# sleep3r/Diffusion-Handwriting-Generation.pytorch

Hardware: AMD Instinct MI355X
Metric: stroke-points/sec reverse-sampled (T=60, L=488) (higher is better)
Workload: dtype bf16; 1 GPU; configs[1]: batch=64 prompts/GPU, T=60, L=488, Lt=30, d_model=128/192/256, num_layers=2, diffusion_mode=new, random-init weights; global_batch=64, seq_len=488, parallelism=batch-shard x1 (no collectives)

## Files before the change

### diffusion-handwriting-generation.pytorch_amd/csrc/convblock_core.h

```cpp
#pragma once
#include <algorithm>
#include "enc_a_core.h"
#include "heads_core.h"

namespace {

#define CB_SILU(x) ((DHW_ABL & 8) ? (x) : silu_t<T>(x))
#define CB_SILU_TILES(NT_, MT_, v) do { if constexpr (!(DHW_ABL & 8)) silu_tiles2<T, NT_, MT_>(v); } while (0)
#define CB_BARRIER() do { if constexpr (!(DHW_ABL & 64)) lds_barrier(); } while (0)

#define STAMP(slot) DHW_STAMP_IF(p.stamps && (int)blockIdx.x == p.stagger && (threadIdx.x & 63) == 0, (threadIdx.x >> 6) * 16 + slot, __builtin_amdgcn_s_memrealtime())

template <typename T, int BM> __host__ __device__ constexpr int h2_stride(int CO) { return BM >= 128 ? CO * (int)sizeof(T) + 16 : tile_stride<T>(CO); }

template <int NT>
struct Epi {
  f32x4 bias[NT], gam[NT], bet[NT];
  DHW_DEV void load(const float* b, const float* g, const float* be, int n0) {
#pragma unroll
    for (int i = 0; i < NT; ++i) {
      bias[i] = *reinterpret_cast<const f32x4*>(b + n0 + 16 * i);
      gam[i] = *reinterpret_cast<const f32x4*>(g + n0 + 16 * i);
      bet[i] = *reinterpret_cast<const f32x4*>(be + n0 + 16 * i);
    }
// ... 4 lines not shown
      bias[i] = *reinterpret_cast<const f32x4*>(b + n0 + 16 * i);
      gam[i] = (f32x4){1, 1, 1, 1};
      bet[i] = (f32x4){0, 0, 0, 0};
    }
  }
};

template <int UPC> constexpr int up_skip_width() { return UPC == 384 ? 256 : UPC == 256 ? 192 : UPC == 192 ? 128 : 0; }
template <typename T, int BM, int CO, int NW, int OCC = 1, int UPC = 0, int CH = 0, int CIN = 0, int TIGHT = 0, int PP = 0, typename P, typename X>
DHW_DEV void convblock_body(const P& p, const X& nx, const int b, const int m0, char* smem) {
  constexpr int ES = sizeof(T), NTHR = NW * 64;
  constexpr bool SK = CIN != 0;
  constexpr int KT1 = 3 * CIN / 32;
  static_assert(UPC == 0 || CIN == 0 || CIN == UPC, "a fused input stage produces the block's own input width");
  constexpr bool ASYM = TIGHT == 2;
  constexpr int BMO = ASYM ? BM : BM - 2 - 2 * TIGHT;
  constexpr int RX = BMO + 4;
  constexpr int BM1 = ASYM ? BM + 16 : BM;
  constexpr int C1 = CO / 2;
  constexpr int T1 = C1 / 16, T2 = CO / 16;
  constexpr int WN1 = NW == 8 ? (T1 >= 8 ? 8 : (T1 == 6 ? 6 : 4)) : 2;
  constexpr int WM1 = NW == 8 ? (T1 >= 6 ? 1 : 2) : 2;
  constexpr bool TALL = NW == 8 && BM >= 128 && T2 == 8;
  constexpr int WN2 = NW == 8 ? (TALL ? 4 : (T2 % 8 == 0 ? 8 : 6)) : 4;
  constexpr int WM2 = TALL ? 2 : 1;
  constexpr int MT1 = BM1 / WM1 / 16, NT1 = T1 / WN1;
  constexpr int MT2 = BM / WM2 / 16, NT2 = T2 / WN2;
  static_assert(NT1 * WN1 == T1 && NT2 * WN2 == T2 && MT1 * 16 * WM1 == BM1 && WM1 * WN1 <= NW && WM2 * WN2 <= NW, "unsupported tile / wave layout");
  static_assert(!ASYM || WM1 == 1, "the asymmetric tiling: blocks with one row group in conv1");
  constexpr bool PPX = PP != 0;
  static_assert(!PPX || (TALL && WM1 == 2 && WN1 == 4 && CH == 0 && !ASYM && OCC == 1), "ping-pong: the 2 x 4 wave layouts of the tall tiles");
  constexpr int RING = (ES == 2 ? 24 : 12) * (CO == 256 ? 2 : 3) / 3 / (OCC * NW > 8 ? OCC : 1);

  const int Ls = sample_len(p.lens, p.lsh, b, p.L);
  if constexpr (DHW_LENS) { if (m0 >= Ls) return; }
  const int tid = body_tid(), lane = tid & 63, wave = __builtin_amdgcn_readfirstlane(tid >> 6);
  const int l15 = lane & 15, g = lane >> 4;
  const int Cin = SK ? CIN : p.Cin;
  const bool pp_lead = PPX && __builtin_amdgcn_readfirstlane(wave) >= NW / 2;
#define PP_BARRIER() do { if constexpr (PPX) CB_BARRIER(); } while (0)

  const int SX = tile_stride<T>(Cin), SH1 = tile_stride<T>(C1), SH2 = h2_stride<T, BM>(CO);
  char* XS = smem;
  char* XR = XS + RX * SX;
  char* H1 = XR + RX * SX;
  char* H2 = H1 + (BM1 + 2) * SH1;
  const float* gam = p.film + (size_t)b * p.film_bs;
  const float* bet = gam + p.film_tot;

  const bool act1 = WM1 * WN1 == NW || wave < WM1 * WN1, act2 = WM2 * WN2 == NW || wave < WM2 * WN2;
  const int wm1 = act1 ? wave / WN1 : 0, wn1 = act1 ? wave % WN1 : 0, row01 = wm1 * (BM1 / WM1), nt01 = wn1 * NT1;
  const int wm2 = act2 ? wave / WN2 : 0, wn2 = act2 ? wave % WN2 : 0, row02 = wm2 * (BM / WM2), nt02 = wn2 * NT2;
  const int n1 = nt01 * 16 + 4 * g, n2 = nt02 * 16 + 4 * g;
  const int KCin = Cin / 32;

  if constexpr (OCC == 2) {
    if (p.stagger && blockIdx.x >= gridDim.x / 2)
      for (int i = 0; i < p.stagger; ++i) __builtin_amdgcn_s_sleep(16);
  }
  STAMP(0);
  WRing<T, NT1, RING> ring1;
  Epi<NT1> ep1;
  auto fill1 = [&]() {
    const T* w = reinterpret_cast<const T*>(p.w_c1) + ((size_t)nt01 * KCin * 3 * 64 + lane) * 8;
    if constexpr (SK) ring1.template fill_s<KT1>(w);
    else ring1.fill(w, KCin * 3);
  };

  if constexpr (UPC != 0) {
    constexpr int RXP = (RX + 15) / 16 * 16, RH = RXP + 2, MTU = RXP / 16;
    constexpr int TU = UPC / 16, WNU = TU % 8 == 0 ? 8 : 4, WMU = NW / WNU, NTU = TU / WNU;
    constexpr int MTG = (MTU + WMU - 1) / WMU;
    static_assert(NTU * WNU == TU && NW == 8, "unsupported input width");
    const int wmu = wave / WNU, wnu = wave % WNU;
    const int ntu0 = wnu * NTU, nu = ntu0 * 16 + 4 * g, rowu0 = wmu * MTG * 16;
    constexpr int UCH = up_skip_width<UPC>();
// ... 115 lines not shown
          const bool k = lrow >= 0 && lrow < Ls;
          uint4 w = make_uint4(k ? v[u].x : 0u, k ? v[u].y : 0u, k ? v[u].z : 0u, k ? v[u].w : 0u);
          *reinterpret_cast<uint4*>(XR + r * SX + cc * 16) = w;
          *reinterpret_cast<uint4*>(XS + r * SX + cc * 16) = (DHW_ABL & 8) ? w : silu_piece<T>(w);
        }
      }
    }
  }
  if (UPC == 0 && act1) {
    fill1();
    ep1.load(p.b_c1, gam + p.f1, bet + p.f1, n1);
  }
  STAMP(15);
  CB_BARRIER();
  if constexpr (PPX) {
    if (!pp_lead) {
      for (int id = tid; id < 2 * SH1 / 16; id += NTHR / 2)
        *reinterpret_cast<uint4*>(H1 + BM1 * SH1 + id * 16) = make_uint4(0, 0, 0, 0);
      CB_BARRIER();
    }
  }
  STAMP(1);

  WRing<T, NT2, RING> ring2;
  Epi<NT2> ep2;

  {
    f32x4 acc[NT1][MT1];
    acc_zero(acc);
    if (act1) {
      if constexpr (SK) ring1.template run_s<MT1, KT1>(acc, XS + (row01 + l15) * SX + g * 8 * ES, SX, KCin);
      else ring1.template run<MT1>(acc, XS + (row01 + l15) * SX + g * 8 * ES, SX, KCin);
    }
    STAMP(2);
    PP_BARRIER();
    constexpr int KT2 = (C1 / 32) * 3;
    const T* w2 = reinterpret_cast<const T*>(p.w_c2) + ((size_t)nt02 * KT2 * 64 + lane) * 8;
    if (act2) { ring2.template fill_begin<KT2>(w2); ep2.load(p.b_c2, gam + p.f2, bet + p.f2, n2); }
    constexpr int ST1 = epilogue_steps<NT1, MT1>(), CH2 = decltype(ring2)::template fill_chunks<KT2>(), PER1 = (CH2 + ST1 - 1) / ST1;
    if (act1) {
      epilogue_pairs<T, NT1, MT1, !(DHW_ABL & 8)>(lane, H1, SH1, row01, n1, acc,
          [&](int i, const f32x4& a) { return (a + ep1.bias[i]) * ep1.gam[i] + ep1.bet[i]; },
          [&](int j) { const int srow = m0 - 1 + row01 + j * 16 + l15; return srow >= 0 && srow < Ls; },
          [](int) { return true; },
          [&](int step) {
            if (act2) {
#pragma unroll
              for (int c = 0; c < PER1; ++c) ring2.template fill_chunk<KT2>(step * PER1 + c);
            }
          });
    } else if (act2) {
#pragma unroll
      for (int c = 0; c < CH2; ++c) ring2.template fill_chunk<KT2>(c);
    }
    if constexpr (!PPX)
    for (int id = tid; id < 2 * SH1 / 16; id += NTHR)
      *reinterpret_cast<uint4*>(H1 + BM1 * SH1 + id * 16) = make_uint4(0, 0, 0, 0);
  }
  STAMP(13);
  CB_BARRIER();
  STAMP(3);

  if (act2) {
    f32x4 acc[NT2][MT2];
    acc_zero(acc);
    ring2.template run_s<MT2, (C1 / 32) * 3>(acc, H1 + (row02 + l15) * SH1 + g * 8 * ES, SH1, C1 / 32);
    STAMP(4);
    PP_BARRIER();
    {
      constexpr int KTF = CO / 32;
      ring2.template fill_begin<KTF>(reinterpret_cast<const T*>(p.w_fc) + ((size_t)nt02 * KTF * 64 + lane) * 8);
      constexpr int ST2 = epilogue_steps<NT2, MT2>(), CHF = decltype(ring2)::template fill_chunks<KTF>(), PER2 = (CHF + ST2 - 1) / ST2;
      epilogue_pairs<T, NT2, MT2, !(DHW_ABL & 8)>(lane, H2, SH2, row02, n2, acc,
          [&](int i, const f32x4& a) { return (a + ep2.bias[i]) * ep2.gam[i] + ep2.bet[i]; },
          [](int) { return true; }, [](int) { return true; },
          [&](int step) {
#pragma unroll
            for (int c = 0; c < PER2; ++c) ring2.template fill_chunk<KTF>(step * PER2 + c);
          });
    }
    ep2.load(p.b_fc, gam + p.f3, bet + p.f3, n2);
  }
  STAMP(14);
  CB_BARRIER();
  STAMP(5);

  f32x4 acc[NT2][MT2];
  acc_zero(acc);
  if (act2) {
    const T* wsk = reinterpret_cast<const T*>(p.w_skip) + ((size_t)nt02 * KCin * 3 * 64 + lane) * 8;
    constexpr bool FCX = SK && CO / 32 <= decltype(ring2)::D && DHW_ABL == 0;
    if constexpr (FCX) ring2.template run_n<MT2, CO / 32, KT1>(acc, H2 + (row02 + l15) * SH2 + g * 8 * ES, SH2, CO / 32, wsk);
    else ring2.template run_s<MT2, CO / 32>(acc, H2 + (row02 + l15) * SH2 + g * 8 * ES, SH2, CO / 32);
    STAMP(6);
    if constexpr (FCX) {}
    else if constexpr (SK) ring2.template fill_s<KT1>(wsk);
    else ring2.fill(wsk, KCin * 3);
#pragma unroll
    for (int i = 0; i < NT2; ++i)
#pragma unroll
      for (int j = 0; j < MT2; ++j) acc[i][j] = (acc[i][j] + ep2.bias[i]) * ep2.gam[i] + ep2.bet[i];
    ep2.load_bias(p.b_skip, n2);
    if constexpr (SK) ring2.template run_s<MT2, KT1>(acc, XR + (row02 + l15 + 1) * SX + g * 8 * ES, SX, KCin);
    else ring2.template run<MT2>(acc, XR + (row02 + l15 + 1) * SX + g * 8 * ES, SX, KCin);
  }
  STAMP(7);
  CB_BARRIER();
  if constexpr (PPX) { if (pp_lead && p.out_f32) CB_BARRIER(); }
  STAMP(8);

  const int rows_valid = min(BMO, Ls - m0);
  if (p.out_f32) {
    constexpr int SO = CO * 4 + 16;
    if (act2) {
#pragma unroll
      for (int i = 0; i < NT2; ++i)
#pragma unroll
        for (int j = 0; j < MT2; ++j)
          store4(reinterpret_cast<float*>(smem + (row02 + j * 16 + l15) * SO) + n2 + 16 * i, acc[i][j] + ep2.bias[i]);
    }
    CB_BARRIER();
    if (p.out)
      tile_copy_out<float>(smem, SO, reinterpret_cast<float*>(p.out) + (size_t)(b * p.L + m0) * CO, CO, rows_valid, CO, tid, NTHR);
    if (p.fuse_heads) {
      const int r = tid >> 2, q = tid & 3;
      float a0 = 0.f, a1 = 0.f, a2 = 0.f;
      if (r < rows_valid) {
        const float* xr = reinterpret_cast<const float*>(smem + r * SO);
#pragma unroll
        for (int c = q * 4; c < CO; c += 16) {
          const f32x4 v = *reinterpret_cast<const f32x4*>(xr + c);
          const f32x4 w0 = *reinterpret_cast<const f32x4*>(p.hp.w_out + c);
          const f32x4 w1 = *reinterpret_cast<const f32x4*>(p.hp.w_out + CO + c);
          const f32x4 w2 = *reinterpret_cast<const f32x4*>(p.hp.w_pen + c);
#pragma unroll
          for (int k = 0; k < 4; ++k) { a0 += v[k] * w0[k]; a1 += v[k] * w1[k]; a2 += v[k] * w2[k]; }
        }
      }
#pragma unroll
      for (int o = 2; o; o >>= 1) {
        a0 += __shfl_xor(a0, o);
        a1 += __shfl_xor(a1, o);
        a2 += __shfl_xor(a2, o);
      }
      if (r < rows_valid && q == 0) heads_finish(p.hp, (long)b * p.L + m0 + r, a0, a1, a2);
    }
  } else {
    if (act2) {
#pragma unroll
      for (int i = 0; i < NT2; ++i)
#pragma unroll
        for (int j = 0; j < MT2; ++j) acc[i][j] += ep2.bias[i];
      store_tiles<T, NT2, MT2>(lane, smem, SH2, row02, n2, acc);
    }
    CB_BARRIER();
    if constexpr (PPX) { if (pp_lead) CB_BARRIER(); }
    if constexpr (!(DHW_ABL & 16))
    tile_copy_out<T>(smem, SH2, reinterpret_cast<T*>(p.out) + (size_t)(b * p.L + m0) * CO, CO, rows_valid, CO, tid, NTHR);
    if (p.pool && !(DHW_ABL & 16))
      tile_copy_out_pool<T>(smem, SH2, reinterpret_cast<T*>(p.pool) + ((size_t)b * (p.L / 2) + m0 / 2) * CO, CO, rows_valid, CO, tid, NTHR);
    if constexpr (CH == 1) {
      static_assert(NW == 8 && sizeof(T) == 2, "enc_a_body runs on 8 waves");
      EncALds m;
      m.XR = smem;
      m.QR = smem + BM * SH2;
      m.red = reinterpret_cast<float*>(m.QR + BM * SH2);
      m.KT = reinterpret_cast<char*>(m.red) + 2 * 8 * BM * sizeof(float);
      m.VT = m.KT + 32 * tile_stride<T>(CO);
      m.VS = smem;
      m.PL = reinterpret_cast<float*>(m.KT + enc_a_text_kv_bytes<T, CO, BM>());
      enc_a_body<T, CO, BM, (ASYM ? 16 : 4)>(nx.a, m, b, m0, rows_valid);
    }
  }
  STAMP(9);
}

template <typename T, int BM, int CO>
// ... 12 lines not shown
```

### diffusion-handwriting-generation.pytorch_amd/csrc/enc_a_core.h

```cpp
#pragma once
#include "attn_core.h"
#include "gemm_core.h"
#include "dhw_kernels.h"

#define ENC_STAMP(slot) do { DHW_STAMP_IF(p.stamps && blockIdx.x == 0 && threadIdx.x == 0, slot, __builtin_amdgcn_s_memrealtime()); \
                             DHW_STAMP_IF(p.stamps && (p.dbg & 4) && blockIdx.x == 0 && (threadIdx.x & 63) == 0, 64 + (threadIdx.x >> 6) * 32 + (slot), __builtin_amdgcn_s_memtime()); } while (0)

template <typename T, int BM>
DHW_DEV void stage_rows(char* dst, int S, const T* src, int C, int b, int L, int m0, int tid, int nthreads) {
  constexpr int ES = sizeof(T);
  const int cpr = C * ES / 16;
  const int total = BM * cpr;
  constexpr int U = 4;
  for (int base = tid; base < total; base += nthreads * U) {
    uint4 v[U];
    int off[U];
#pragma unroll
    for (int u = 0; u < U; ++u) {
      const int id = base + u * nthreads;
      const int r = id / cpr, cc = id - r * cpr;
      v[u] = make_uint4(0, 0, 0, 0);
      off[u] = id < total ? r * S + cc * 16 : -1;
      if (id < total && m0 + r < L)
        v[u] = *reinterpret_cast<const uint4*>(reinterpret_cast<const char*>(src) + ((size_t)(b * L + m0 + r) * C) * ES + (size_t)cc * 16);
// ... 67 lines not shown
      if (c < W / 4 && grp + 4 < NS) *reinterpret_cast<uint4*>(pa + 4 * W) = b;
    }
  }
};
template <typename T> constexpr bool enc_plds() { return sizeof(T) == 2; }
template <typename T, int DM> constexpr size_t enc_a_param_bytes() { return enc_plds<T>() ? (size_t)7 * DM * sizeof(float) : 0; }

struct EncALds {
  char* XR;
  char* QR;
  float* red;
  char* KT;
  char* VT;
  char* VS;
  float* PL;
};
template <typename T, int DM, int BM>
constexpr size_t enc_a_text_kv_bytes() {
  return sizeof(T) == 2 ? (size_t)2 * 32 * tile_stride<T>(DM) : (size_t)32 * tile_stride<T>(DM) + (size_t)DM * (32 * sizeof(T) + OPAD<T>);
}
template <typename T, int DM> constexpr int qkv_stride() { return sizeof(T) == 2 ? 3 * DM : 2 * DM; }

template <int DM> constexpr int enc_wn() { return DM % 128 == 0 ? 8 : 6; }

template <typename T, int DM, int BM, int VPIECE = 16, typename P>
DHW_DEV void enc_a_body(const P& p, const EncALds& m, int b, int m0, int rows_valid) {
  constexpr int ES = sizeof(T);
  constexpr int WN = enc_wn<DM>(), WM = 1;
  constexpr int MT = BM / WM / 16, NT = DM / WN / 16, H = DM / 64, KC = DM / 32;
  static_assert(NT * WN * 16 == DM, "channel tiles must divide over the waves");
  const int tid = body_tid(), lane = tid & 63, wave = tid >> 6;
  const int l15 = lane & 15, g = lane >> 4;
  const bool act = WN * WM == 8 || wave < WN * WM;
  const int wm = act ? wave / WN : 0, wn = act ? wave % WN : 0;
  const int S = tile_stride<T>(DM);
  const int Ls = sample_len(p.lens, p.lsh, b, p.Lk);
  char* XR = m.XR;
  char* QR = m.QR;
  float* red = m.red;
  const float* gam = p.film + (size_t)b * p.film_bs;
  const float* bet = gam + p.film_tot;
  const int row0 = wm * (BM / WM), ntile0 = wn * NT;
  const int n0 = ntile0 * 16 + 4 * g;
  const size_t wlane = ((size_t)ntile0 * KC * 64 + lane) * 8;
  const char* xop = XR + (row0 + l15) * S + g * 8 * ES;
  const char* qop = QR + (row0 + l15) * S + g * 8 * ES;

  constexpr int RINGA = sizeof(T) == 4 ? 12 : 24;
  typedef WRing<T, NT, RINGA, (RINGA + NT - 1) / NT> RingT;
  RingT ring;
  constexpr bool SPREADA = sizeof(T) == 2;
  constexpr bool SPREADQ = sizeof(T) == 2 && MT > 1;
  constexpr int FCHA = RingT::template fill_chunks<KC>(), FQA = (FCHA + 3) / 4;
  EpiParams<NT> ep;
  ENC_STAMP(0);
  constexpr bool VROW = sizeof(T) == 2;
  constexpr int KBC = 32, SKC = tile_stride<T>(DM), SVC = VROW ? SKC : KBC * ES + OPAD<T>;
  constexpr int EPV = 16 / ES, CPR = DM / EPV, PPR = KBC / EPV;
  constexpr int UX = (BM * CPR + 511) / 512, UK = (KBC * CPR + 511) / 512, UV = VROW ? UK : (DM * PPR + 511) / 512;
  constexpr int QKS = qkv_stride<T, DM>();
  char* KT = m.KT;
  char* VT = m.VT;
  const T* k1s = reinterpret_cast<const T*>(p.k1) + (size_t)b * p.Lt * DM;
  const T* v1s = reinterpret_cast<const T*>(p.vt1) + (VROW ? (size_t)b * p.Lt * DM : (size_t)b * DM * p.lpadT);
  constexpr bool PLDS = enc_plds<T>();
  const float* PL = m.PL;
  const int64_t* trow = p.text ? p.text + (size_t)b * p.Lt : nullptr;
  PadMask<KBC> pad;
  struct KVRegs { CopyRegs<UK> ck; CopyRegs<UV> cv; };
  auto kv_store = [&](KVRegs& kv) {
    CopyRegs<UK>& ck = kv.ck;
    CopyRegs<UV>& cv = kv.cv;
    ck.store(KBC * CPR, tid, 512, [&](int id) { const int r = id / CPR, cc = id - r * CPR; return reinterpret_cast<uint4*>(KT + r * SKC + cc * 16); },
             [&](int id) { return id / CPR < p.Lt; });
    if constexpr (VROW)
      cv.store(KBC * CPR, tid, 512, [&](int id) { const int r = id / CPR, cc = id - r * CPR; return reinterpret_cast<uint4*>(VT + r * SVC + cc * 16); },
               [&](int id) { return id / CPR < p.Lt; });
// ... 10 lines not shown
    ParamStage<7> cp;
    if constexpr (PLDS) {
      cp.template load<DM>(tid, p.b_q1, p.b_d1, gam + p.f1, bet + p.f1, p.b_qkv2, p.b_qkv2 + DM, p.b_qkv2 + 2 * DM);
    }
    const T* xs = reinterpret_cast<const T*>(p.x);
    if (p.x)
      cx.load(BM * CPR, tid, 512, [&](int id) { const int r = id / CPR, cc = id - r * CPR;
                                                return reinterpret_cast<const uint4*>(xs + (size_t)(b * p.Lk + (m0 + r < p.Lk ? m0 + r : p.Lk - 1)) * DM + cc * EPV); });
    ck.load(KBC * CPR, tid, 512, [&](int id) { const int r = id / CPR, cc = id - r * CPR;
                                               return reinterpret_cast<const uint4*>(k1s + (size_t)(r < p.Lt ? r : p.Lt - 1) * DM + cc * EPV); });
    if constexpr (VROW)
      cv.load(KBC * CPR, tid, 512, [&](int id) { const int r = id / CPR, cc = id - r * CPR;
                                                 return reinterpret_cast<const uint4*>(v1s + (size_t)(r < p.Lt ? r : p.Lt - 1) * DM + cc * EPV); });
    else
      cv.load(DM * PPR, tid, 512, [&](int id) { const int ch = id / PPR, part = id - ch * PPR;
                                                return reinterpret_cast<const uint4*>(v1s + (size_t)ch * p.lpadT + ((part + 1) * EPV <= p.lpadT ? part * EPV : 0)); });
    if (p.x)
      cx.store(BM * CPR, tid, 512, [&](int id) { const int r = id / CPR, cc = id - r * CPR; return reinterpret_cast<uint4*>(XR + r * S + cc * 16); },
               [&](int id) { return m0 + id / CPR < Ls; });
    kv_store(kv);
    if constexpr (PLDS) cp.template store<DM>(m.PL, tid);
  }
  pad.load(lane, trow, 0, p.Lt);
  if (act) {
    ring.template fill_s<KC>(reinterpret_cast<const T*>(p.w_q1) + wlane);
    if constexpr (!PLDS) ep.load_bias(p.b_q1, n0);
  }
  lds_barrier();
  ENC_STAMP(1);

  if (act) {
    f32x4 acc[NT][MT];
    acc_zero(acc);
    f32x4 pb[NT][MT];
#pragma unroll
    for (int i = 0; i < NT; ++i)
#pragma unroll
      for (int j = 0; j < MT; ++j)
        pb[i][j] = *reinterpret_cast<const f32x4*>(p.pb_q1 + (unsigned)((m0 + row0 + j * 16 + l15) * DM + n0 + 16 * i));
    ring.template run_s<MT, KC>(acc, xop, S, KC);
    ENC_STAMP(8);
    if constexpr (PLDS) ep.lds_bias(PL, n0);
#pragma unroll
    for (int i = 0; i < NT; ++i)
#pragma unroll
      for (int j = 0; j < MT; ++j) acc[i][j] += ep.bias[i] + pb[i][j];
    enc_store_tiles<T, NT, MT>(lane, QR, S, row0, n0, acc);
    ENC_STAMP(9);
  }
  lds_barrier();
  ENC_STAMP(2);

  {
    constexpr int RG = BM / 16, HS = 8 / RG, UMAX = (H + HS - 1) / HS;
    constexpr int SK = SKC, SV = SVC;
    const int rg = wave % RG, hs = wave / RG;
    Frag<T> qf[UMAX][2];
    float mr[UMAX], lr[UMAX];
    f32x4 o[UMAX][4];
#pragma unroll
    for (int u = 0; u < UMAX; ++u) {
      const int h = hs + u * HS;
      const T* qrow = reinterpret_cast<const T*>(QR + (rg * 16 + l15) * S) + (h < H ? h : 0) * 64 + 8 * g;
      qf[u][0] = frag_load(qrow);
      qf[u][1] = frag_load(qrow + 32);
      mr[u] = -INFINITY;
      lr[u] = 0.f;
#pragma unroll
      for (int t = 0; t < 4; ++t) o[u][t] = (f32x4){0, 0, 0, 0};
    }
    for (int kb = 0; kb < p.Lt; kb += KBC) {
      if (kb) pad.load(lane, trow, kb, p.Lt);
      const unsigned padbits = pad.template bits<sizeof(T) == 2>();
      if (kb) {
        attn_stage_kv<T, KBC>(KT, SK, VT, SV, k1s, DM, v1s, VROW ? DM : p.lpadT, DM, kb, p.Lt, tid, 512);
        lds_barrier();
      }
      attn_units<T, KBC, true, UMAX>(lane, qf, KT, SK, VT, SV, hs, HS, H, kb, padbits, p.Lt, mr, lr, o);
      if (kb + KBC < p.Lt) lds_barrier();
    }
#pragma unroll
    for (int u = 0; u < UMAX; ++u) {
      const int h = hs + u * HS;
      float l = lr[u];
      l = xg_sum(l);
      const float inv = 1.0f / l;
      if (h < H) {
        T* dst = reinterpret_cast<T*>(QR + (rg * 16 + l15) * S) + h * 64 + 4 * g;
        store_pair(lane, dst, dst + 16, o[u][0] * inv, o[u][1] * inv);
        store_pair(lane, dst + 32, dst + 48, o[u][2] * inv, o[u][3] * inv);
      }
    }
  }
  if (act) {
    ring.template fill_s<KC>(reinterpret_cast<const T*>(p.w_d1) + wlane);
    if constexpr (!PLDS) ep.load(p.b_d1, gam + p.f1, bet + p.f1, n0);
  }
  lds_barrier();
  ENC_STAMP(3);

  {
    f32x4 acc[NT][MT];
    acc_zero(acc);
    if (act) {
      ring.template run_s<MT, KC>(acc, qop, S, KC);
      ENC_STAMP(10);
      if constexpr (SPREADA) { ring.template fill_begin<KC>(reinterpret_cast<const T*>(p.w_qkv2) + wlane); ring.template fill_range<KC, 0, FQA>(); }
      else ring.template fill_s<KC>(reinterpret_cast<const T*>(p.w_qkv2) + wlane);
      if constexpr (PLDS) ep.lds(PL + DM, PL + 2 * DM, PL + 3 * DM, n0);
#pragma unroll
      for (int i = 0; i < NT; ++i)
#pragma unroll
        for (int j = 0; j < MT; ++j) acc[i][j] += ep.bias[i];
      if constexpr (SPREADA) ring.template fill_range<KC, FQA, 2 * FQA>();
    }
    if constexpr (SPREADA) ln_rows<T, MT, NT, WN, BM>(acc, red, wn, row0, lane, DM, act, [&]() { if (act) ring.template fill_range<KC, 2 * FQA, 3 * FQA>(); });
// ... 85 lines not shown
#pragma unroll
            for (int k = 0; k < 4; ++k)
              *reinterpret_cast<T*>(VS + (n0 + 16 * i + k) * SV + rl * ES) = from_f<T>(rl < rows_valid ? v[k] : 0.f);
          }
      }
      lds_barrier();
      constexpr int KPP = VPIECE / ES, PPR = BM / KPP;
      const int klimit = m0 + rows_valid >= Ls ? min(BM, p.lpadX - m0) : rows_valid;
      for (int id = tid; id < DM * PPR; id += 512) {
        const int ch = id / PPR, part = id - ch * PPR;
        if ((part + 1) * KPP <= klimit) {
          T* dst = reinterpret_cast<T*>(p.vt2) + ((size_t)b * DM + ch) * p.lpadX + m0 + part * KPP;
          const char* src = VS + ch * SV + part * VPIECE;
          if constexpr (VPIECE == 16) *reinterpret_cast<uint4*>(dst) = *reinterpret_cast<const uint4*>(src);
          else *reinterpret_cast<uint32_t*>(dst) = *reinterpret_cast<const uint32_t*>(src);
        }
      }
    }
    ENC_STAMP(5 + chunk);
  };
  qkv_chunk(std::integral_constant<int, 0>{});
  qkv_chunk(std::integral_constant<int, 1>{});
  qkv_chunk(std::integral_constant<int, 2>{});
}
```

### diffusion-handwriting-generation.pytorch_amd/csrc/enc_bc_core.h

```cpp
#pragma once
#include "enc_a_core.h"

namespace {

#define STAMP(slot) ENC_STAMP(slot)
#ifdef DHW_STAMPS
#define WST(slot) do { if (p.stamps && blockIdx.x == 0 && lane == 0) p.stamps[64 + wave * 32 + (slot)] = __builtin_amdgcn_s_memtime(); } while (0)
#else
#define WST(slot) do { } while (0)
#endif

template <typename T, int DM, int BM, typename P>
DHW_DEV void enc_a_tile(const P& p, const int b, const int m0, char* smem) {
  const int S = tile_stride<T>(DM);
  EncALds m;
  m.XR = smem;
  m.QR = m.XR + BM * S;
  m.red = reinterpret_cast<float*>(m.QR + BM * S);
  m.KT = reinterpret_cast<char*>(m.red) + 2 * 8 * BM * sizeof(float);
  m.VT = m.KT + 32 * tile_stride<T>(DM);
  m.VS = smem;
  m.PL = reinterpret_cast<float*>(m.KT + enc_a_text_kv_bytes<T, DM, BM>());
  const int Ls = sample_len(p.lens, p.lsh, b, p.Lk);
  if constexpr (DHW_LENS) { if (m0 >= Ls) return; }
// ... 18 lines not shown
}
template <typename T, int DM> constexpr size_t enc_bc_param_bytes() { return enc_plds<T>() ? (size_t)8 * DM * sizeof(float) : 0; }
template <typename T, int DM, int BM>
constexpr bool bc_params_fixed() { return lds_bc_tiles<T, DM, BM>() + enc_bc_param_bytes<T, DM>() <= 160 * 1024; }
template <typename T, int DM, int BM>
constexpr size_t lds_bc_bytes() { return lds_bc_tiles<T, DM, BM>() + (bc_params_fixed<T, DM, BM>() ? enc_bc_param_bytes<T, DM>() : 0); }

template <typename T, int DM, int BM, int NEXT>
constexpr size_t lds_bc_chain_bytes() {
  constexpr size_t S = tile_stride<T>(DM), base = 3 * BM * S + 2 * 8 * BM * sizeof(float);
  constexpr size_t chain = NEXT == 1 ? base + enc_a_text_kv_bytes<T, DM, BM>() + enc_a_param_bytes<T, DM>()
                         : NEXT == 2 ? base + enc_a_text_kv_bytes<T, 384, BM / 2>() + enc_a_param_bytes<T, 384>() : 0;
  return chain > lds_bc_bytes<T, DM, BM>() ? chain : lds_bc_bytes<T, DM, BM>();
}

template <typename T, int DM, int BM>
constexpr size_t lds_a_bytes() { return (size_t)2 * BM * tile_stride<T>(DM) + 2 * 8 * BM * sizeof(float) + enc_a_text_kv_bytes<T, DM, BM>() + enc_a_param_bytes<T, DM>(); }

template <typename T, int DM, int BM, int NEXT = 0, typename P, typename X>
DHW_DEV void enc_bc_body(const P& p, const X& nx, const int b, const int m0, char* smem) {
  constexpr int ES = sizeof(T);
  const int Ls = sample_len(p.lens, p.lsh, b, p.Lk);
  if constexpr (DHW_LENS) { if (m0 >= Ls) return; }
  constexpr int WN = enc_wn<DM>(), WM = 1;
  constexpr int MT = BM / WM / 16, NT = DM / WN / 16, H = DM / 64, KC = DM / 32;
  constexpr int RING = sizeof(T) == 4 ? 12 : (DM == 384 && BM >= 32 ? 15 : 24), RDMAX = (RING + NT - 1) / NT;
  const int tid = body_tid(), lane = tid & 63, wave = tid >> 6;
  const int l15 = lane & 15, g = lane >> 4;
  const bool act = WN * WM == 8 || wave < WN * WM;
  const int wm = act ? wave / WN : 0, wn = act ? wave % WN : 0;
  const int S = tile_stride<T>(DM);
  char* R1 = smem;
  char* R2 = R1 + BM * S;
  char* R3 = R2 + BM * S;
  float* red = reinterpret_cast<float*>(R3 + BM * S);
  const float* gam = p.film + (size_t)b * p.film_bs;
  const float* bet = gam + p.film_tot;
  const int row0 = wm * (BM / WM), ntile0 = wn * NT;
  const int n0 = ntile0 * 16 + 4 * g;
  const size_t wlane = ((size_t)ntile0 * KC * 64 + lane) * 8;
  const char* op1 = R1 + (row0 + l15) * S + g * 8 * ES;
  const char* op3 = R3 + (row0 + l15) * S + g * 8 * ES;

  WRing<T, NT, RING, RDMAX> ring;
  constexpr bool SPREAD = sizeof(T) == 2;
  constexpr int FCH = WRing<T, NT, RING, RDMAX>::template fill_chunks<KC>(), FQ = (FCH + 3) / 4;
  EpiParams<NT> ep;
  constexpr bool PLDS = enc_plds<T>(), PLFIX = bc_params_fixed<T, DM, BM>();
  float* PL = reinterpret_cast<float*>(smem + lds_bc_tiles<T, DM, BM>());
  ParamStage<8> cp;
#define BC_PARAMS_REQUEST() cp.template load<DM>(tid, p.b_d2, gam + p.f2, bet + p.f2, p.b_f1, p.b_f1 + DM, p.b_f2, gam + p.f3, bet + p.f3)
  STAMP(16);
  WST(0);
  DHW_STAMP_IF(p.stamps && blockIdx.x == 0 && threadIdx.x == 0, 40, __builtin_amdgcn_s_memtime());
  if (!(p.dbg & 1)) {
    constexpr int RG = BM / 16, HS = 8 / RG, UMAX = (H + HS - 1) / HS, KBS = self_kbs<T, DM, BM>();
    constexpr bool DB = self_db<T, DM, BM>();
    constexpr bool VROW = sizeof(T) == 2;
    constexpr int SK = tile_stride<T>(DM), SV = VROW ? SK : KBS * ES + self_vpad<T, DM, BM>();
    constexpr int BUFB = KBS * SK + (VROW ? KBS * SV : DM * SV);
    constexpr int QKS = qkv_stride<T, DM>();
    const int rg = wave % RG, hs = wave / RG;
    auto unit_head = [&](int u) { return hs + u * HS; };
    const T* qk = reinterpret_cast<const T*>(p.qk2);
    const T* ksrc = qk + (size_t)b * p.Lk * QKS + DM;
    const T* vsrc = VROW ? ksrc + DM : reinterpret_cast<const T*>(p.vt2) + (size_t)b * DM * p.lpadX;
    constexpr int EPV = 16 / ES, CPR = DM / EPV, PPR = KBS / EPV;
    constexpr int UK = (KBS * CPR + 511) / 512, UV = VROW ? UK : (DM * PPR + 511) / 512;
    CopyRegs<UK> ck;
    CopyRegs<UV> cv;
// ... 61 lines not shown
      static_assert((size_t)2 * BM * tile_stride<T>(DM) + 2 * 8 * BM * sizeof(float) + enc_bc_param_bytes<T, DM>() <= (size_t)BUFB, "parameter block inside buffer 0");
      PL = reinterpret_cast<float*>(((ib - 1) & 1) ? R2 + 2 * BM * S + 2 * 8 * BM * sizeof(float) : R2 + BUFB);
      cp.template store<DM>(PL, tid);
    }
    WST(1);
#pragma unroll
    for (int u = 0; u < UMAX; ++u) {
      const int h = unit_head(u);
      float l = lr[u];
      l = xg_sum(l);
      const float inv = 1.0f / l;
      if (h < H) {
        T* dst = reinterpret_cast<T*>(R1 + (rg * 16 + l15) * S) + h * 64 + 4 * g;
        store_pair(lane, dst, dst + 16, o[u][0] * inv, o[u][1] * inv);
        store_pair(lane, dst + 32, dst + 48, o[u][2] * inv, o[u][3] * inv);
      }
    }
  }
  else if constexpr (PLDS) {
    BC_PARAMS_REQUEST();
    if constexpr (!PLFIX) PL = reinterpret_cast<float*>(R2 + 2 * BM * S + 2 * 8 * BM * sizeof(float));
    cp.template store<DM>(PL, tid);
  }
  if (act) {
    ring.template fill_s<KC>(reinterpret_cast<const T*>(p.w_d2) + wlane);
    if constexpr (!PLDS) ep.load(p.b_d2, gam + p.f2, bet + p.f2, n0);
  }
  WST(2);
  lds_barrier();
  WST(3);
  STAMP(17);

  {
    f32x4 acc[NT][MT];
    acc_zero(acc);
    if (act) {
      f32x4 res[NT][MT];
#pragma unroll
      for (int i = 0; i < NT; ++i)
#pragma unroll
        for (int j = 0; j < MT; ++j) {
          const int r = m0 + row0 + j * 16 + l15;
          res[i][j] = load4(reinterpret_cast<const T*>(p.x2) + (unsigned)((b * p.Lk + r) * DM + n0 + 16 * i));
        }
      ring.template run_s<MT, KC>(acc, op1, S, KC);
      WST(4);
// ... 65 lines not shown
    if (hh == 0) lds_barrier();
    WST(15 + 6 * hh);
    STAMP(21 + 2 * hh);
  }
  if (act) {
    if constexpr (PLDS) ep.lds(PL + 5 * DM, PL + 6 * DM, PL + 7 * DM, n0);
    else ep.load(p.b_f2, gam + p.f3, bet + p.f3, n0);
#pragma unroll
    for (int i = 0; i < NT; ++i)
#pragma unroll
      for (int j = 0; j < MT; ++j)
        acc2[i][j] += ep.bias[i] + load4(reinterpret_cast<const T*>(R2 + (row0 + j * 16 + l15) * S) + n0 + 16 * i);
  }
  WST(22);
  ln_rows<T, MT, NT, WN, BM>(acc2, red, wn, row0, lane, DM, act);
  WST(23);
  if (act) {
#pragma unroll
    for (int i = 0; i < NT; ++i)
#pragma unroll
      for (int j = 0; j < MT; ++j) acc2[i][j] = acc2[i][j] * ep.gam[i] + ep.bet[i];
    enc_store_tiles<T, NT, MT>(lane, R3, S, row0, n0, acc2);
  }
  lds_barrier();
  const int rows_valid = min(BM, Ls - m0);
  tile_copy_out<T>(R3, S, reinterpret_cast<T*>(p.out) + (size_t)(b * p.Lk + m0) * DM, DM, rows_valid, DM, tid, 512);
  if (p.pool)
    tile_copy_out_pool<T>(R3, S, reinterpret_cast<T*>(p.pool) + ((size_t)b * (p.Lk / 2) + m0 / 2) * DM, DM, rows_valid, DM, tid, 512);
  STAMP(24);
  WST(24);
  DHW_STAMP_IF(p.stamps && blockIdx.x == 0 && threadIdx.x == 0, 41, __builtin_amdgcn_s_memtime());

  if constexpr (NEXT == 1) {
    EncALds m;
    m.XR = R3; m.QR = R1; m.red = red;
    m.KT = reinterpret_cast<char*>(red) + 2 * 8 * BM * sizeof(float);
    m.VT = m.KT + 32 * tile_stride<T>(DM);
    m.VS = R1;
    m.PL = reinterpret_cast<float*>(m.KT + enc_a_text_kv_bytes<T, DM, BM>());
    enc_a_body<T, DM, BM>(nx.a, m, b, m0, rows_valid);
  } else if constexpr (NEXT == 2) {
    constexpr int DN = 384, BN2 = BM / 2, SN = tile_stride<T>(DN), NTN = DN / 8 / 16, MTN = BN2 / 16;
    {
      constexpr int EPV = 16 / ES;
      const int cpr = DM / EPV;
      for (int id = tid; id < BN2 * cpr; id += 512) {
// ... 43 lines not shown
```

Before: 1.826 million stroke-points/s.

## Spread 192-channel tiles over all eight waves with uneven per-wave widths

For 192-channel layers (12 channel tiles), the conv block's second stage and the encoder bodies previously used 6 waves with 2 tiles each, leaving 2 of 8 waves idle. The new code gives waves 0-3 two tiles and waves 4-7 one tile each, dispatching through a templated lambda so each wave runs a compile-time tile count with its own weight ring. All eight waves now do work in those stages. The price is imbalance, since the two-tile waves still set the critical path, plus code duplication, register-pressure changes and smaller rings for the single-tile waves.

Result: no change. 1.840 million stroke-points/s (median of 6 runs) (+0.8%).

```diff
diff --git a/diffusion-handwriting-generation.pytorch_amd/csrc/convblock_core.h b/diffusion-handwriting-generation.pytorch_amd/csrc/convblock_core.h
--- a/diffusion-handwriting-generation.pytorch_amd/csrc/convblock_core.h
+++ b/diffusion-handwriting-generation.pytorch_amd/csrc/convblock_core.h
@@ -50,11 +50,12 @@
   constexpr int WN1 = NW == 8 ? (T1 >= 8 ? 8 : (T1 == 6 ? 6 : 4)) : 2;
   constexpr int WM1 = NW == 8 ? (T1 >= 6 ? 1 : 2) : 2;
   constexpr bool TALL = NW == 8 && BM >= 128 && T2 == 8;
-  constexpr int WN2 = NW == 8 ? (TALL ? 4 : (T2 % 8 == 0 ? 8 : 6)) : 4;
+  constexpr bool L21 = NW == 8 && !TALL && T2 == 12 && OCC == 1;
+  constexpr int WN2 = NW == 8 ? (TALL ? 4 : (T2 % 8 == 0 || L21 ? 8 : 6)) : 4;
   constexpr int WM2 = TALL ? 2 : 1;
   constexpr int MT1 = BM1 / WM1 / 16, NT1 = T1 / WN1;
-  constexpr int MT2 = BM / WM2 / 16, NT2 = T2 / WN2;
-  static_assert(NT1 * WN1 == T1 && NT2 * WN2 == T2 && MT1 * 16 * WM1 == BM1 && WM1 * WN1 <= NW && WM2 * WN2 <= NW, "unsupported tile / wave layout");
+  constexpr int MT2 = BM / WM2 / 16, NT2U = L21 ? 2 : T2 / WN2;
+  static_assert(NT1 * WN1 == T1 && (L21 || NT2U * WN2 == T2) && MT1 * 16 * WM1 == BM1 && WM1 * WN1 <= NW && WM2 * WN2 <= NW, "unsupported tile / wave layout");
   static_assert(!ASYM || WM1 == 1, "the asymmetric tiling: blocks with one row group in conv1");
   constexpr bool PPX = PP != 0;
   static_assert(!PPX || (TALL && WM1 == 2 && WN1 == 4 && CH == 0 && !ASYM && OCC == 1), "ping-pong: the 2 x 4 wave layouts of the tall tiles");
@@ -78,8 +79,8 @@
 
   const bool act1 = WM1 * WN1 == NW || wave < WM1 * WN1, act2 = WM2 * WN2 == NW || wave < WM2 * WN2;
   const int wm1 = act1 ? wave / WN1 : 0, wn1 = act1 ? wave % WN1 : 0, row01 = wm1 * (BM1 / WM1), nt01 = wn1 * NT1;
-  const int wm2 = act2 ? wave / WN2 : 0, wn2 = act2 ? wave % WN2 : 0, row02 = wm2 * (BM / WM2), nt02 = wn2 * NT2;
-  const int n1 = nt01 * 16 + 4 * g, n2 = nt02 * 16 + 4 * g;
+  const int wm2 = act2 ? wave / WN2 : 0, wn2 = act2 ? wave % WN2 : 0, row02 = wm2 * (BM / WM2);
+  const int n1 = nt01 * 16 + 4 * g;
   const int KCin = Cin / 32;
 
   if constexpr (OCC == 2) {
@@ -241,103 +242,129 @@
   }
   STAMP(1);
 
-  WRing<T, NT2, RING> ring2;
-  Epi<NT2> ep2;
-
-  {
-    f32x4 acc[NT1][MT1];
-    acc_zero(acc);
-    if (act1) {
-      if constexpr (SK) ring1.template run_s<MT1, KT1>(acc, XS + (row01 + l15) * SX + g * 8 * ES, SX, KCin);
-      else ring1.template run<MT1>(acc, XS + (row01 + l15) * SX + g * 8 * ES, SX, KCin);
-    }
-    STAMP(2);
-    PP_BARRIER();
-    constexpr int KT2 = (C1 / 32) * 3;
-    const T* w2 = reinterpret_cast<const T*>(p.w_c2) + ((size_t)nt02 * KT2 * 64 + lane) * 8;
-    if (act2) { ring2.template fill_begin<KT2>(w2); ep2.load(p.b_c2, gam + p.f2, bet + p.f2, n2); }
-    constexpr int ST1 = epilogue_steps<NT1, MT1>(), CH2 = decltype(ring2)::template fill_chunks<KT2>(), PER1 = (CH2 + ST1 - 1) / ST1;
-    if (act1) {
-      epilogue_pairs<T, NT1, MT1, !(DHW_ABL & 8)>(lane, H1, SH1, row01, n1, acc,
-          [&](int i, const f32x4& a) { return (a + ep1.bias[i]) * ep1.gam[i] + ep1.bet[i]; },
-          [&](int j) { const int srow = m0 - 1 + row01 + j * 16 + l15; return srow >= 0 && srow < Ls; },
-          [](int) { return true; },
-          [&](int step) {
-            if (act2) {
-#pragma unroll
-              for (int c = 0; c < PER1; ++c) ring2.template fill_chunk<KT2>(step * PER1 + c);
-            }
-          });
-    } else if (act2) {
-#pragma unroll
-      for (int c = 0; c < CH2; ++c) ring2.template fill_chunk<KT2>(c);
-    }
-    if constexpr (!PPX)
-    for (int id = tid; id < 2 * SH1 / 16; id += NTHR)
-      *reinterpret_cast<uint4*>(H1 + BM1 * SH1 + id * 16) = make_uint4(0, 0, 0, 0);
-  }
-  STAMP(13);
-  CB_BARRIER();
-  STAMP(3);
-
-  if (act2) {
+  f32x4 acc1[NT1][MT1];
+  acc_zero(acc1);
+  if (act1) {
+    if constexpr (SK) ring1.template run_s<MT1, KT1>(acc1, XS + (row01 + l15) * SX + g * 8 * ES, SX, KCin);
+    else ring1.template run<MT1>(acc1, XS + (row01 + l15) * SX + g * 8 * ES, SX, KCin);
+  }
+  STAMP(2);
+  PP_BARRIER();
+
+  const int rows_valid = min(BMO, Ls - m0);
+  const bool act1_rt = act1;
+  auto stages23 = [&](auto NT2_, auto A1_, const int nt02) __attribute__((always_inline)) {
+    constexpr int NT2 = decltype(NT2_)::value;
+    const bool act1 = decltype(A1_)::value == 2 ? act1_rt : decltype(A1_)::value == 1;
+    const int n2 = nt02 * 16 + 4 * g;
+    WRing<T, NT2, RING> ring2;
+    Epi<NT2> ep2;
+    {
+      constexpr int KT2 = (C1 / 32) * 3;
+      const T* w2 = reinterpret_cast<const T*>(p.w_c2) + ((size_t)nt02 * KT2 * 64 + lane) * 8;
+      if (act2) { ring2.template fill_begin<KT2>(w2); ep2.load(p.b_c2, gam + p.f2, bet + p.f2, n2); }
+      constexpr int ST1 = epilogue_steps<NT1, MT1>(), CH2 = decltype(ring2)::template fill_chunks<KT2>(), PER1 = (CH2 + ST1 - 1) / ST1;
+      if (act1) {
+        epilogue_pairs<T, NT1, MT1, !(DHW_ABL & 8)>(lane, H1, SH1, row01, n1, acc1,
+            [&](int i, const f32x4& a) { return (a + ep1.bias[i]) * ep1.gam[i] + ep1.bet[i]; },
+            [&](int j) { const int srow = m0 - 1 + row01 + j * 16 + l15; return srow >= 0 && srow < Ls; },
+            [](int) { return true; },
+            [&](int step) {
+              if (act2) {
+#pragma unroll
+                for (int c = 0; c < PER1; ++c) ring2.template fill_chunk<KT2>(step * PER1 + c);
+              }
+            });
+      } else if (act2) {
+#pragma unroll
+        for (int c = 0; c < CH2; ++c) ring2.template fill_chunk<KT2>(c);
+      }
+      if constexpr (!PPX)
+      for (int id = tid; id < 2 * SH1 / 16; id += NTHR)
+        *reinterpret_cast<uint4*>(H1 + BM1 * SH1 + id * 16) = make_uint4(0, 0, 0, 0);
+    }
+    STAMP(13);
+    CB_BARRIER();
+    STAMP(3);
+
+    if (act2) {
+      f32x4 acc[NT2][MT2];
+      acc_zero(acc);
+      ring2.template run_s<MT2, (C1 / 32) * 3>(acc, H1 + (row02 + l15) * SH1 + g * 8 * ES, SH1, C1 / 32);
+      STAMP(4);
+      PP_BARRIER();
+      {
+        constexpr int KTF = CO / 32;
+        ring2.template fill_begin<KTF>(reinterpret_cast<const T*>(p.w_fc) + ((size_t)nt02 * KTF * 64 + lane) * 8);
+        constexpr int ST2 = epilogue_steps<NT2, MT2>(), CHF = decltype(ring2)::template fill_chunks<KTF>(), PER2 = (CHF + ST2 - 1) / ST2;
+        epilogue_pairs<T, NT2, MT2, !(DHW_ABL & 8)>(lane, H2, SH2, row02, n2, acc,
+            [&](int i, const f32x4& a) { return (a + ep2.bias[i]) * ep2.gam[i] + ep2.bet[i]; },
+            [](int) { return true; }, [](int) { return true; },
+            [&](int step) {
+#pragma unroll
+              for (int c = 0; c < PER2; ++c) ring2.template fill_chunk<KTF>(step * PER2 + c);
+            });
+      }
+      ep2.load(p.b_fc, gam + p.f3, bet + p.f3, n2);
+    }
+    STAMP(14);
+    CB_BARRIER();
+    STAMP(5);
+
     f32x4 acc[NT2][MT2];
     acc_zero(acc);
-    ring2.template run_s<MT2, (C1 / 32) * 3>(acc, H1 + (row02 + l15) * SH1 + g * 8 * ES, SH1, C1 / 32);
-    STAMP(4);
-    PP_BARRIER();
-    {
-      constexpr int KTF = CO / 32;
-      ring2.template fill_begin<KTF>(reinterpret_cast<const T*>(p.w_fc) + ((size_t)nt02 * KTF * 64 + lane) * 8);
-      constexpr int ST2 = epilogue_steps<NT2, MT2>(), CHF = decltype(ring2)::template fill_chunks<KTF>(), PER2 = (CHF + ST2 - 1) / ST2;
-      epilogue_pairs<T, NT2, MT2, !(DHW_ABL & 8)>(lane, H2, SH2, row02, n2, acc,
-          [&](int i, const f32x4& a) { return (a + ep2.bias[i]) * ep2.gam[i] + ep2.bet[i]; },
-          [](int) { return true; }, [](int) { return true; },
-          [&](int step) {
-#pragma unroll
-            for (int c = 0; c < PER2; ++c) ring2.template fill_chunk<KTF>(step * PER2 + c);
-          });
-    }
-    ep2.load(p.b_fc, gam + p.f3, bet + p.f3, n2);
-  }
-  STAMP(14);
-  CB_BARRIER();
-  STAMP(5);
-
-  f32x4 acc[NT2][MT2];
-  acc_zero(acc);
-  if (act2) {
-    const T* wsk = reinterpret_cast<const T*>(p.w_skip) + ((size_t)nt02 * KCin * 3 * 64 + lane) * 8;
-    constexpr bool FCX = SK && CO / 32 <= decltype(ring2)::D && DHW_ABL == 0;
-    if constexpr (FCX) ring2.template run_n<MT2, CO / 32, KT1>(acc, H2 + (row02 + l15) * SH2 + g * 8 * ES, SH2, CO / 32, wsk);
-    else ring2.template run_s<MT2, CO / 32>(acc, H2 + (row02 + l15) * SH2 + g * 8 * ES, SH2, CO / 32);
-    STAMP(6);
-    if constexpr (FCX) {}
-    else if constexpr (SK) ring2.template fill_s<KT1>(wsk);
-    else ring2.fill(wsk, KCin * 3);
-#pragma unroll
-    for (int i = 0; i < NT2; ++i)
-#pragma unroll
-      for (int j = 0; j < MT2; ++j) acc[i][j] = (acc[i][j] + ep2.bias[i]) * ep2.gam[i] + ep2.bet[i];
-    ep2.load_bias(p.b_skip, n2);
-    if constexpr (SK) ring2.template run_s<MT2, KT1>(acc, XR + (row02 + l15 + 1) * SX + g * 8 * ES, SX, KCin);
-    else ring2.template run<MT2>(acc, XR + (row02 + l15 + 1) * SX + g * 8 * ES, SX, KCin);
-  }
-  STAMP(7);
-  CB_BARRIER();
-  if constexpr (PPX) { if (pp_lead && p.out_f32) CB_BARRIER(); }
-  STAMP(8);
-
-  const int rows_valid = min(BMO, Ls - m0);
+    if (act2) {
+      const T* wsk = reinterpret_cast<const T*>(p.w_skip) + ((size_t)nt02 * KCin * 3 * 64 + lane) * 8;
+      constexpr bool FCX = SK && CO / 32 <= decltype(ring2)::D && DHW_ABL == 0;
+      if constexpr (FCX) ring2.template run_n<MT2, CO / 32, KT1>(acc, H2 + (row02 + l15) * SH2 + g * 8 * ES, SH2, CO / 32, wsk);
+      else ring2.template run_s<MT2, CO / 32>(acc, H2 + (row02 + l15) * SH2 + g * 8 * ES, SH2, CO / 32);
+      STAMP(6);
+      if constexpr (FCX) {}
+      else if constexpr (SK) ring2.template fill_s<KT1>(wsk);
+      else ring2.fill(wsk, KCin * 3);
+#pragma unroll
+      for (int i = 0; i < NT2; ++i)
+#pragma unroll
+        for (int j = 0; j < MT2; ++j) acc[i][j] = (acc[i][j] + ep2.bias[i]) * ep2.gam[i] + ep2.bet[i];
+      ep2.load_bias(p.b_skip, n2);
+      if constexpr (SK) ring2.template run_s<MT2, KT1>(acc, XR + (row02 + l15 + 1) * SX + g * 8 * ES, SX, KCin);
+      else ring2.template run<MT2>(acc, XR + (row02 + l15 + 1) * SX + g * 8 * ES, SX, KCin);
+    }
+    STAMP(7);
+    CB_BARRIER();
+    if constexpr (PPX) { if (pp_lead && p.out_f32) CB_BARRIER(); }
+    STAMP(8);
+
+    if (p.out_f32) {
+      constexpr int SO = CO * 4 + 16;
+      if (act2) {
+#pragma unroll
+        for (int i = 0; i < NT2; ++i)
+#pragma unroll
+          for (int j = 0; j < MT2; ++j)
+            store4(reinterpret_cast<float*>(smem + (row02 + j * 16 + l15) * SO) + n2 + 16 * i, acc[i][j] + ep2.bias[i]);
+      }
+    } else {
+      if (act2) {
+#pragma unroll
+        for (int i = 0; i < NT2; ++i)
+#pragma unroll
+          for (int j = 0; j < MT2; ++j) acc[i][j] += ep2.bias[i];
+        store_tiles<T, NT2, MT2>(lane, smem, SH2, row02, n2, acc);
+      }
+    }
+  };
+  if constexpr (L21) {
+    static_assert(WM1 == 1 && WN1 == 6, "conv1 of the 192-channel blocks: one channel tile on each of waves 0-5");
+    if (wave < 4) stages23(std::integral_constant<int, 2>{}, std::integral_constant<int, 1>{}, 2 * wave);
+    else if (wave < 6) stages23(std::integral_constant<int, 1>{}, std::integral_constant<int, 1>{}, 4 + wave);
+    else stages23(std::integral_constant<int, 1>{}, std::integral_constant<int, 0>{}, 4 + wave);
+  } else {
+    stages23(std::integral_constant<int, NT2U>{}, std::integral_constant<int, 2>{}, wn2 * NT2U);
+  }
+
   if (p.out_f32) {
     constexpr int SO = CO * 4 + 16;
-    if (act2) {
-#pragma unroll
-      for (int i = 0; i < NT2; ++i)
-#pragma unroll
-        for (int j = 0; j < MT2; ++j)
-          store4(reinterpret_cast<float*>(smem + (row02 + j * 16 + l15) * SO) + n2 + 16 * i, acc[i][j] + ep2.bias[i]);
-    }
     CB_BARRIER();
     if (p.out)
       tile_copy_out<float>(smem, SO, reinterpret_cast<float*>(p.out) + (size_t)(b * p.L + m0) * CO, CO, rows_valid, CO, tid, NTHR);
@@ -365,13 +392,6 @@
       if (r < rows_valid && q == 0) heads_finish(p.hp, (long)b * p.L + m0 + r, a0, a1, a2);
     }
   } else {
-    if (act2) {
-#pragma unroll
-      for (int i = 0; i < NT2; ++i)
-#pragma unroll
-        for (int j = 0; j < MT2; ++j) acc[i][j] += ep2.bias[i];
-      store_tiles<T, NT2, MT2>(lane, smem, SH2, row02, n2, acc);
-    }
     CB_BARRIER();
     if constexpr (PPX) { if (pp_lead) CB_BARRIER(); }
     if constexpr (!(DHW_ABL & 16))
diff --git a/diffusion-handwriting-generation.pytorch_amd/csrc/enc_a_core.h b/diffusion-handwriting-generation.pytorch_amd/csrc/enc_a_core.h
--- a/diffusion-handwriting-generation.pytorch_amd/csrc/enc_a_core.h
+++ b/diffusion-handwriting-generation.pytorch_amd/csrc/enc_a_core.h
@@ -113,14 +113,26 @@
 template <typename T, int DM> constexpr int qkv_stride() { return sizeof(T) == 2 ? 3 * DM : 2 * DM; }
 
 template <int DM> constexpr int enc_wn() { return DM % 128 == 0 ? 8 : 6; }
+template <typename T, int DM> constexpr bool enc_l21() { return sizeof(T) == 2 && DM == 192; }
+template <typename T, int DM, typename Part>
+DHW_DEV void enc_dispatch(int wave, Part part) {
+  if constexpr (enc_l21<T, DM>()) {
+    if (wave < 4) part(std::integral_constant<int, 2>{}, 2 * wave);
+    else part(std::integral_constant<int, 1>{}, 4 + wave);
+  } else {
+    constexpr int WN = enc_wn<DM>(), NT = DM / WN / 16;
+    part(std::integral_constant<int, NT>{}, wave < WN ? wave * NT : 0);
+  }
+}
 
 template <typename T, int DM, int BM, int VPIECE = 16, typename P>
 DHW_DEV void enc_a_body(const P& p, const EncALds& m, int b, int m0, int rows_valid) {
   constexpr int ES = sizeof(T);
-  constexpr int WN = enc_wn<DM>(), WM = 1;
-  constexpr int MT = BM / WM / 16, NT = DM / WN / 16, H = DM / 64, KC = DM / 32;
-  static_assert(NT * WN * 16 == DM, "channel tiles must divide over the waves");
-  const int tid = body_tid(), lane = tid & 63, wave = tid >> 6;
+  constexpr bool L21 = enc_l21<T, DM>();
+  constexpr int WN = L21 ? 8 : enc_wn<DM>(), WM = 1;
+  constexpr int MT = BM / WM / 16, H = DM / 64, KC = DM / 32;
+  static_assert(L21 || DM / WN / 16 * WN * 16 == DM, "channel tiles must divide over the waves");
+  const int tid = body_tid(), lane = tid & 63, wave = L21 ? __builtin_amdgcn_readfirstlane(tid >> 6) : tid >> 6;
   const int l15 = lane & 15, g = lane >> 4;
   const bool act = WN * WM == 8 || wave < WN * WM;
   const int wm = act ? wave / WN : 0, wn = act ? wave % WN : 0;
@@ -131,19 +143,21 @@
   float* red = m.red;
   const float* gam = p.film + (size_t)b * p.film_bs;
   const float* bet = gam + p.film_tot;
-  const int row0 = wm * (BM / WM), ntile0 = wn * NT;
-  const int n0 = ntile0 * 16 + 4 * g;
-  const size_t wlane = ((size_t)ntile0 * KC * 64 + lane) * 8;
+  const int row0 = wm * (BM / WM);
   const char* xop = XR + (row0 + l15) * S + g * 8 * ES;
   const char* qop = QR + (row0 + l15) * S + g * 8 * ES;
 
-  constexpr int RINGA = sizeof(T) == 4 ? 12 : 24;
-  typedef WRing<T, NT, RINGA, (RINGA + NT - 1) / NT> RingT;
-  RingT ring;
   constexpr bool SPREADA = sizeof(T) == 2;
   constexpr bool SPREADQ = sizeof(T) == 2 && MT > 1;
-  constexpr int FCHA = RingT::template fill_chunks<KC>(), FQA = (FCHA + 3) / 4;
-  EpiParams<NT> ep;
+#define ENC_A_WAVE_TILES()                                                                                                                     \
+  constexpr int NT = decltype(NT_)::value;                                                                                                     \
+  const int n0 = ntile0 * 16 + 4 * g;                                                                         \
+  const size_t wlane = ((size_t)ntile0 * KC * 64 + lane) * 8;                       \
+  constexpr int RINGA = sizeof(T) == 4 ? 12 : (L21 ? 12 * NT : 24);    \
+  typedef WRing<T, NT, RINGA, (RINGA + NT - 1) / NT> RingT;                                                                                    \
+  constexpr int FCHA = RingT::template fill_chunks<KC>(), FQA = (FCHA + 3) / 4;                                                                \
+  RingT ring;                                                                                                                                  \
+  EpiParams<NT> ep
   ENC_STAMP(0);
   constexpr bool VROW = sizeof(T) == 2;
   constexpr int KBC = 32, SKC = tile_stride<T>(DM), SVC = VROW ? SKC : KBC * ES + OPAD<T>;
@@ -200,6 +214,8 @@
     if constexpr (PLDS) cp.template store<DM>(m.PL, tid);
   }
   pad.load(lane, trow, 0, p.Lt);
+  enc_dispatch<T, DM>(wave, [&](auto NT_, const int ntile0) __attribute__((always_inline)) {
+  ENC_A_WAVE_TILES();
   if (act) {
     ring.template fill_s<KC>(reinterpret_cast<const T*>(p.w_q1) + wlane);
     if constexpr (!PLDS) ep.load_bias(p.b_q1, n0);
@@ -226,6 +242,7 @@
     enc_store_tiles<T, NT, MT>(lane, QR, S, row0, n0, acc);
     ENC_STAMP(9);
   }
+  });
   lds_barrier();
   ENC_STAMP(2);
 
@@ -270,6 +287,8 @@
       }
     }
   }
+  enc_dispatch<T, DM>(wave, [&](auto NT_, const int ntile0) __attribute__((always_inline)) {
+  ENC_A_WAVE_TILES();
   if (act) {
     ring.template fill_s<KC>(reinterpret_cast<const T*>(p.w_d1) + wlane);
     if constexpr (!PLDS) ep.load(p.b_d1, gam + p.f1, bet + p.f1, n0);
@@ -401,4 +420,6 @@
   qkv_chunk(std::integral_constant<int, 0>{});
   qkv_chunk(std::integral_constant<int, 1>{});
   qkv_chunk(std::integral_constant<int, 2>{});
+  });
+#undef ENC_A_WAVE_TILES
 }
diff --git a/diffusion-handwriting-generation.pytorch_amd/csrc/enc_bc_core.h b/diffusion-handwriting-generation.pytorch_amd/csrc/enc_bc_core.h
--- a/diffusion-handwriting-generation.pytorch_amd/csrc/enc_bc_core.h
+++ b/diffusion-handwriting-generation.pytorch_amd/csrc/enc_bc_core.h
@@ -64,10 +64,10 @@
   constexpr int ES = sizeof(T);
   const int Ls = sample_len(p.lens, p.lsh, b, p.Lk);
   if constexpr (DHW_LENS) { if (m0 >= Ls) return; }
-  constexpr int WN = enc_wn<DM>(), WM = 1;
-  constexpr int MT = BM / WM / 16, NT = DM / WN / 16, H = DM / 64, KC = DM / 32;
-  constexpr int RING = sizeof(T) == 4 ? 12 : (DM == 384 && BM >= 32 ? 15 : 24), RDMAX = (RING + NT - 1) / NT;
-  const int tid = body_tid(), lane = tid & 63, wave = tid >> 6;
+  constexpr bool L21 = enc_l21<T, DM>();
+  constexpr int WN = L21 ? 8 : enc_wn<DM>(), WM = 1;
+  constexpr int MT = BM / WM / 16, H = DM / 64, KC = DM / 32;
+  const int tid = body_tid(), lane = tid & 63, wave = L21 ? __builtin_amdgcn_readfirstlane(tid >> 6) : tid >> 6;
   const int l15 = lane & 15, g = lane >> 4;
   const bool act = WN * WM == 8 || wave < WN * WM;
   const int wm = act ? wave / WN : 0, wn = act ? wave % WN : 0;
@@ -78,16 +78,11 @@
   float* red = reinterpret_cast<float*>(R3 + BM * S);
   const float* gam = p.film + (size_t)b * p.film_bs;
   const float* bet = gam + p.film_tot;
-  const int row0 = wm * (BM / WM), ntile0 = wn * NT;
-  const int n0 = ntile0 * 16 + 4 * g;
-  const size_t wlane = ((size_t)ntile0 * KC * 64 + lane) * 8;
+  const int row0 = wm * (BM / WM);
   const char* op1 = R1 + (row0 + l15) * S + g * 8 * ES;
   const char* op3 = R3 + (row0 + l15) * S + g * 8 * ES;
 
-  WRing<T, NT, RING, RDMAX> ring;
   constexpr bool SPREAD = sizeof(T) == 2;
-  constexpr int FCH = WRing<T, NT, RING, RDMAX>::template fill_chunks<KC>(), FQ = (FCH + 3) / 4;
-  EpiParams<NT> ep;
   constexpr bool PLDS = enc_plds<T>(), PLFIX = bc_params_fixed<T, DM, BM>();
   float* PL = reinterpret_cast<float*>(smem + lds_bc_tiles<T, DM, BM>());
   ParamStage<8> cp;
@@ -195,6 +190,14 @@
     if constexpr (!PLFIX) PL = reinterpret_cast<float*>(R2 + 2 * BM * S + 2 * 8 * BM * sizeof(float));
     cp.template store<DM>(PL, tid);
   }
+  enc_dispatch<T, DM>(wave, [&](auto NT_, const int ntile0) __attribute__((always_inline)) {
+  constexpr int NT = decltype(NT_)::value;
+  const int n0 = ntile0 * 16 + 4 * g;
+  const size_t wlane = ((size_t)ntile0 * KC * 64 + lane) * 8;
+  constexpr int RING = sizeof(T) == 4 ? 12 : (DM == 384 && BM >= 32 ? 15 : (L21 ? 12 * NT : 24)), RDMAX = (RING + NT - 1) / NT;
+  WRing<T, NT, RING, RDMAX> ring;
+  constexpr int FCH = WRing<T, NT, RING, RDMAX>::template fill_chunks<KC>(), FQ = (FCH + 3) / 4;
+  EpiParams<NT> ep;
   if (act) {
     ring.template fill_s<KC>(reinterpret_cast<const T*>(p.w_d2) + wlane);
     if constexpr (!PLDS) ep.load(p.b_d2, gam + p.f2, bet + p.f2, n0);
@@ -306,6 +309,7 @@
       for (int j = 0; j < MT; ++j) acc2[i][j] = acc2[i][j] * ep.gam[i] + ep.bet[i];
     enc_store_tiles<T, NT, MT>(lane, R3, S, row0, n0, acc2);
   }
+  });
   lds_barrier();
   const int rows_valid = min(BM, Ls - m0);
   tile_copy_out<T>(R3, S, reinterpret_cast<T*>(p.out) + (size_t)(b * p.Lk + m0) * DM, DM, rows_valid, DM, tid, 512);
```
